# felixchenfy/Monocular-Visual-Odometry

Hardware: AMD Instinct MI355X
Metric: frames/sec (extract+match+5-kf BA), 640x480 / 2000 kp, 1->8 MI355X (higher is better)
Workload: dtype u8 (extract/match) + f64 (BA); 1 GPU

## Files before the change

monocular-visual-odometry_amd/csrc/ba_kernels.hip:

```cpp
#include "ba_types.h"
#include "mvo_internal.h"

typedef ba_u64 u64;
#ifndef MVO_KERNEL_SIM
typedef __attribute__((address_space(1))) double gdouble;
typedef __attribute__((address_space(1))) const u64 gcu64;
typedef __attribute__((address_space(1))) u64 gu64;
#define BA_AS_GLOBAL_D(p) ((gdouble*)(p))
#define BA_AS_GLOBAL_CU64(p) ((gcu64*)(p))
#define BA_AS_GLOBAL_U64(p) ((gu64*)(p))
#else
typedef double gdouble;
typedef const u64 gcu64;
typedef u64 gu64;
#define BA_AS_GLOBAL_D(p) (p)
#define BA_AS_GLOBAL_CU64(p) (p)
#define BA_AS_GLOBAL_U64(p) (p)
#endif

#define PH_BEGIN() long long ph_t = PROF ? (long long)__builtin_amdgcn_s_memtime() : 0
#define PH_END(id)                                                       \
    do {                                                                 \
        if (PROF) {                                                      \
            long long ph_n = (long long)__builtin_amdgcn_s_memtime();    \
// ... 344 lines not shown
    for (int o = 32; o > 0; o >>= 1) v = min(v, __shfl_xor(v, o));
    return v;
#endif
}

__device__ __forceinline__ int group_sum_i(int v, int width) {
#ifndef MVO_KERNEL_SIM
    v += __builtin_amdgcn_update_dpp(0, v, 0xb1, 0xf, 0xf, false);
    v += __builtin_amdgcn_update_dpp(0, v, 0x4e, 0xf, 0xf, false);
    if (width >= 8) v += __builtin_amdgcn_update_dpp(0, v, 0x141, 0xf, 0xf, false);
    if (width >= 16) v += __builtin_amdgcn_update_dpp(0, v, 0x140, 0xf, 0xf, false);
    return v;
#else
    for (int o = 1; o < width; o <<= 1) v += __shfl_xor(v, o);
    return v;
#endif
}

__device__ __attribute__((noinline)) void ba_pivot_replay(const short* rank, int n, short* perm, int lane) {
    const int done = 0x7fffffff;
    if (n <= 64) {
        int rk = lane < n ? (int)rank[lane] : -1, el = lane, out = 0, cur = 0;
        for (int k = 0; k < n; ++k) {
            const unsigned long long fresh = __ballot(rk == k), running = __ballot(rk == cur);
            const unsigned long long m = fresh ? fresh : running;
            cur = fresh ? k : cur;
            const int big = m ? (int)__builtin_ctzll(m) : k;
            const int kr = __builtin_amdgcn_readlane(rk, k), ke = __builtin_amdgcn_readlane(el, k), eb = __builtin_amdgcn_readlane(el, big);
            rk = lane == big ? kr : rk;
            el = lane == big ? ke : el;
            rk = lane == k ? -1 : rk;
            out = lane == k ? eb : out;
        }
        if (lane < n) perm[lane] = (short)out;
        return;
    }
    const int p0 = lane, p1 = lane + 64;
    int k0 = p0 < n ? ((int)rank[p0] << 7) | p0 : done, k1 = p1 < n ? ((int)rank[p1] << 7) | p1 : done;
    int e0 = p0, e1 = p1;
    for (int k = 0; k < n; ++k) {
        const int big = wave_min_i(min(k0, k1)) & 127;
        const int ek = k < 64 ? __builtin_amdgcn_readlane(e0, k) : __builtin_amdgcn_readlane(e1, k - 64);
        const int kk = k < 64 ? __builtin_amdgcn_readlane(k0, k) : __builtin_amdgcn_readlane(k1, k - 64);
        const int eb = big < 64 ? __builtin_amdgcn_readlane(e0, big) : __builtin_amdgcn_readlane(e1, big - 64);
        const int kmoved = (kk & ~127) | big;
        if (p0 == big) e0 = ek, k0 = kmoved;
        if (p1 == big) e1 = ek, k1 = kmoved;
        if (p0 == k) e0 = eb, k0 = done;
        if (p1 == k) e1 = eb, k1 = done;
    }
    if (p0 < n) perm[p0] = (short)e0;
    if (p1 < n) perm[p1] = (short)e1;
}

#include "ba_solve.h"

__device__ __attribute__((noinline)) double ba_stale_scale_landmarks(gcu64* dxl, int bl_off, int Lg, double lambda, int lane) {
    const double* bl = ba_dyn_lds + bl_off;
    double sp = 0;
    for (int l0 = lane; l0 < Lg; l0 += 4 * 64) {
        double xs[4][3];
#pragma unroll
        for (int u = 0; u < 4; ++u)
#pragma unroll
            for (int c = 0; c < 3; ++c) {
                const int l = l0 + 64 * u;
                xs[u][c] = l < Lg ? __longlong_as_double((long long)__hip_atomic_load(dxl + 3 * l + c, __ATOMIC_RELAXED, __HIP_MEMORY_SCOPE_AGENT)) : 0.0;
            }
#pragma unroll
        for (int u = 0; u < 4; ++u) {
            const int l = l0 + 64 * u;
            if (l < Lg) {
#pragma unroll
                for (int c = 0; c < 3; ++c) sp += xs[u][c] * (lambda * xs[u][c] + bl[3 * l + c]);
            }
        }
    }
    return wave_sum_d(sp);
}


__device__ __attribute__((noinline)) int solve_lds(int sl_off, int cb_off, int n, int lane) {
    double* S = ba_dyn_lds + sl_off;
    double* col = ba_dyn_lds + cb_off;
    const int ld = n + 2;
    int ok = 1;
    for (int j = 0; j < n; ++j) {
        const double d = S[j * ld + j];
        if (!(d >= BA_PIVOT_MIN && d <= BA_PIVOT_MAX)) {
            ok = 0;
            break;
        }
        const double r = ba_rcp_pivot(d);
        for (int i = j + 1 + lane; i <= n; i += 64) col[i] = S[i * ld + j];
        __builtin_amdgcn_wave_barrier();
        for (int i = j + 1 + lane; i <= n; i += 64) {
            const double l = col[i] * r;
            const int kend = i < n ? i : n - 1;
            for (int k = j + 1; k <= kend; ++k) S[i * ld + k] = __builtin_fma(-l, col[k], S[i * ld + k]);
            S[i * ld + j] = l;
        }
        __builtin_amdgcn_wave_barrier();
    }
    if (ok) {
        for (int j = lane; j < n; j += 64) col[j] = S[n * ld + j];
        __builtin_amdgcn_wave_barrier();
        for (int i = n - 1; i >= 1; --i) {
            const double xi = col[i];
            for (int j = lane; j < i; j += 64) col[j] = __builtin_fma(-S[i * ld + j], xi, col[j]);
            __builtin_amdgcn_wave_barrier();
        }
    }
    return ok;
}

__device__ __forceinline__ void packed_ij(int idx, int n, int& i, int& j) {
    const int ntri = n * (n + 1) / 2;
    if (idx < ntri) {
        i = (int)((sqrt(8.0 * idx + 1.0) - 1.0) * 0.5);
        while (i * (i + 1) / 2 > idx) --i;
        while ((i + 1) * (i + 2) / 2 <= idx) ++i;
        j = idx - i * (i + 1) / 2;
    } else {
        i = n;
        j = idx - ntri;
    }
}

struct WgLds {
    double* SL;
    double* colbuf;
    double* pan;
    double* Rl;
    double* hpl;
    double* uv;
    double* uvg;
    double* pts;
    double* bak;
    double* Hll;
    double* bl;
    double* Cc;
    double* cl;
    double* dxl;
    double* U;
    double* E2;
    short* epose;
    short* ept;
    short* dup;
    short* ptl;
    short* pti;
    short* pts0;
    short* eof;
};

__device__ __forceinline__ double edge_error(const BaDev& B, const WgLds& W, int el, const double* sR,
                                             const double* sT, double* Xc, double* ew) {
    const int p = W.epose[el], l = W.ept[el];
    const double* R = sR + 9 * p;
    const double* t = sT + 3 * p;
    const double X0 = W.pts[3 * l], X1 = W.pts[3 * l + 1], X2 = W.pts[3 * l + 2];
    Xc[0] = R[0] * X0 + R[1] * X1 + R[2] * X2 + t[0];
    Xc[1] = R[3] * X0 + R[4] * X1 + R[5] * X2 + t[1];
    Xc[2] = R[6] * X0 + R[7] * X1 + R[8] * X2 + t[2];
    const double mu = B.uv_global ? W.uvg[2 * el] : W.uv[el], mv = B.uv_global ? W.uvg[2 * el + 1] : W.uv[B.maxEg + el];
    const double e0 = mu - (Xc[0] / Xc[2] * B.f + B.cx);
    const double e1 = mv - (Xc[1] / Xc[2] * B.f + B.cy);
    ew[0] = B.lc00 * e0 + B.lc01 * e1;
    ew[1] = B.lc11 * e1;
    return ew[0] * ew[0] + ew[1] * ew[1];
}

__device__ double robust_chi2_local(const BaDev& B, const WgLds& W, int Eg, const double* sR, const double* sT,
                                    double* scratch) {
    double s = 0;
    for (int el = threadIdx.x; el < Eg; el += BA_THREADS) {
        double Xc[3], ew[2], r0, r1;
        huber(edge_error(B, W, el, sR, sT, Xc, ew), B.delta, r0, r1);
        s += r0;
    }
    return block_sum(s, scratch);
}

__device__ __forceinline__ int u_index(int col, int row, int ldu) {
    return col * ldu + row;
}

template <int LDU>
__device__ __forceinline__ v4d schur_chain_t(const double* U, int ti, int tj, int m0, int m1, int lane) {
    v4d acc = {0, 0, 0, 0};
    const int k = lane >> 4, i = lane & 15;
    constexpr int st = 4 * LDU;
    const double* pa = U + (size_t)(4 * m0 + k) * LDU + (16 * ti + i);
    const double* pb = U + (size_t)(4 * m0 + k) * LDU + (16 * tj + i);
    int m = m0;
#define BA_LOAD4(A, Bv) \
    A##0 = pa[0], Bv##0 = pb[0], A##1 = pa[st], Bv##1 = pb[st], A##2 = pa[2 * st], Bv##2 = pb[2 * st], A##3 = pa[3 * st], Bv##3 = pb[3 * st]; \
    pa += 4 * st;                                                                                                                           \
    pb += 4 * st
#define BA_MFMA4_LOADNEXT(A, Bv, C, D, more)                                     \
    acc = __builtin_amdgcn_mfma_f64_16x16x4f64(A##0, Bv##0, acc, 0, 0, 0);       \
    __builtin_amdgcn_sched_barrier(0);                                           \
    if (more) { BA_LOAD4(C, D); }                                                \
    __builtin_amdgcn_sched_barrier(0);                                           \
    acc = __builtin_amdgcn_mfma_f64_16x16x4f64(A##1, Bv##1, acc, 0, 0, 0);       \
    acc = __builtin_amdgcn_mfma_f64_16x16x4f64(A##2, Bv##2, acc, 0, 0, 0);       \
    acc = __builtin_amdgcn_mfma_f64_16x16x4f64(A##3, Bv##3, acc, 0, 0, 0)
    if (m + 4 <= m1) {
        double a0, a1, a2, a3, b0, b1, b2, b3, c0 = 0, c1 = 0, c2 = 0, c3 = 0, d0 = 0, d1 = 0, d2 = 0, d3 = 0;
        BA_LOAD4(a, b);
        m += 4;
        for (;;) {
            const bool more1 = m + 4 <= m1;
            BA_MFMA4_LOADNEXT(a, b, c, d, more1);
            if (!more1) break;
            m += 4;
            const bool more2 = m + 4 <= m1;
            BA_MFMA4_LOADNEXT(c, d, a, b, more2);
            if (!more2) break;
            m += 4;
        }
    }
#undef BA_LOAD4
#undef BA_MFMA4_LOADNEXT
    for (; m < m1; ++m) {
        acc = __builtin_amdgcn_mfma_f64_16x16x4f64(pa[0], pb[0], acc, 0, 0, 0);
        pa += st;
        pb += st;
    }
    return acc;
}
__device__ __forceinline__ v4d schur_chain(const double* U, int ldu, int ti, int tj, int m0, int m1, int lane) {
    switch (ldu) {
        case 17: return schur_chain_t<17>(U, ti, tj, m0, m1, lane);
        case 33: return schur_chain_t<33>(U, ti, tj, m0, m1, lane);
        case 49: return schur_chain_t<49>(U, ti, tj, m0, m1, lane);
        case 65: return schur_chain_t<65>(U, ti, tj, m0, m1, lane);
        default: break;
    }
    v4d acc = {0, 0, 0, 0};
    const int k = lane >> 4, i = lane & 15;
    const double* pa = U + (size_t)(4 * m0 + k) * ldu + (16 * ti + i);
    const double* pb = U + (size_t)(4 * m0 + k) * ldu + (16 * tj + i);
    for (int m = m0; m < m1; ++m) {
        acc = __builtin_amdgcn_mfma_f64_16x16x4f64(pa[0], pb[0], acc, 0, 0, 0);
        pa += 4 * ldu;
        pb += 4 * ldu;
    }
    return acc;
}

struct EdgeRegs {
    double a0[6], a1[6];
    double x[6];
};
__device__ __forceinline__ void edge_Y(const EdgeRegs& r, const double* cc, double* Y) {
    const double c0 = cc[0], c1 = cc[1], c2 = cc[2], c3 = cc[3], c4 = cc[4], c5 = cc[5];
    Y[0] = r.x[0] * c0 + r.x[1] * c1 + r.x[2] * c3;
    Y[1] = r.x[1] * c2 + r.x[2] * c4;
    Y[2] = r.x[2] * c5;
    Y[3] = r.x[3] * c0 + r.x[4] * c1 + r.x[5] * c3;
    Y[4] = r.x[4] * c2 + r.x[5] * c4;
    Y[5] = r.x[5] * c5;
}

struct BaRun {
    unsigned tag0;
    int use_mfma, same_l2_ok;
};
template <bool PROF, int NR, int SLOTS>
__device__ __forceinline__ void ba_window(const BaDev* desc, const BaRun batch, const int g) {
    __shared__ BaDev sB;
    {
        const unsigned* src = reinterpret_cast<const unsigned*>(desc);
        unsigned* dst = reinterpret_cast<unsigned*>(&sB);
        for (unsigned i = threadIdx.x; i < sizeof(BaDev) / 4; i += BA_THREADS) dst[i] = src[i];
    }
    __syncthreads();
    const BaDev& B = sB;
    if (g >= B.G) return;
    const unsigned long long t_begin = __builtin_amdgcn_s_memrealtime();
    double* dyn = ba_dyn_lds;
    __shared__ double sScr[BA_WAVES];
    double* const sP = dyn;
    double* const sPbak = sP + 8 * B.F;
    double* const sR = sPbak + 8 * B.F;
    double* const sT = sR + 9 * B.F;
    double* const sHpp = sT + 3 * B.F;
    double* const sBp = sHpp + 36 * B.F;
    double* const sDx = sBp + 6 * B.F;
    double* const sSol = sDx + 6 * B.F;
    double* const sX = dyn + ba_pose_doubles(B.F);
    __shared__ int sSlot[BA_MAX_POSES], sSlotPose[BA_MAX_POSES], sPoseStart[BA_MAX_POSES + 1];
    __shared__ short sSlc[3][BA_HP_PASSES][BA_MAX_POSES];
    __shared__ int sFlag[6];
    __shared__ double sStale[BA_WAVES + 2];
    __shared__ short sPermAll[2][6 * BA_MAX_POSES];
    short* const sPerm = sPermAll[0];
    __shared__ short sRank[6 * BA_MAX_POSES];
    short* const sPermTie = sPermAll[1];
    __shared__ long long sStamp[PROF ? 32 : 1];
    if (threadIdx.x == 0) sFlag[1] = sFlag[2] = sFlag[3] = sFlag[4] = 0;
    if (threadIdx.x < 6 * BA_MAX_POSES) sRank[threadIdx.x] = -1;
    int tid = threadIdx.x, lane = tid & 63;
#define BA_PHASE_HEAD()            \
    do {                           \
        tid = ba_fresh_i(tid);     \
        lane = tid & 63;           \
    } while (0)
    const int wave = __builtin_amdgcn_readfirstlane(tid >> 6);
    const int n = B.n, G = B.G, nfree = B.nfree, urows = B.ldu, ldu = B.ldu + 1, nlow = B.nlow, npk = B.npk;
    const int pt_lo = B.wg_pt_start[g], Lg = B.wg_pt_start[g + 1] - pt_lo;
    const int e_lo = B.wg_edge_start[g], Eg = B.wg_edge_start[g + 1] - e_lo;
    const unsigned tag0 = batch.tag0;
    unsigned tagA = 0, tagB = 0, tagH = 0;

    WgLds W;
    double* stage;
    {
        double* d = dyn + ba_pose_doubles(B.F) + 2 * (size_t)G + 8;
        W.SL = d;
        d += ba_solver_doubles(n, nlow + B.nhp, G, B.npair, B.npar, B.panel, B.alias_sl) - 3 * 64 - (B.panel ? BA_PANEL_DOUBLES : 0);
        W.colbuf = d;
        d += 3 * 64;
        W.pan = d;
        d += B.panel ? BA_PANEL_DOUBLES : 0;
        W.Rl = d;
        d += nlow + B.nhp + 16;
        W.hpl = d;
        d += B.nhp + 1;
        W.uv = d;
        d += B.uv_global ? 0 : (size_t)B.maxEg * 2;
        W.uvg = B.uv_dev + 2 * (size_t)e_lo;
        W.pts = d;
        d += (size_t)B.maxLg * 3;
        const size_t full = B.fix_points ? 0 : 1;
        W.bak = d;
        d += full * B.maxLg * 3;
        W.Hll = d;
        d += full * B.maxLg * BA_XS;
        W.bl = d;
        d += full * B.maxLg * 3;
        W.Cc = d;
        d += full * B.maxLg * BA_XS;
        W.cl = d;
        d += full * B.maxLg * 3;
        W.dxl = B.dxl_dev + 3 * (size_t)pt_lo;
        W.U = d;
        stage = d;
        if (B.alias_sl) W.SL = d;
        d += B.uarea;
        W.E2 = d;
        d += (size_t)B.e2_edges * BA_E2S;
        short* s = reinterpret_cast<short*>(d);
        W.epose = s;
        s += B.maxEg;
        W.ept = s;
        s += B.maxEg;
        W.dup = s;
        s += B.maxEg;
        W.ptl = s;
        s += B.maxEg;
        W.pti = s;
        s += B.maxEg;
        W.pts0 = s;
        s += B.maxLg + 1;
        W.eof = s;
    }
    for (int el = tid; el < Eg; el += BA_THREADS) {
        W.epose[el] = (short)B.e_pose[e_lo + el];
        W.ept[el] = (short)(B.e_point[e_lo + el] - pt_lo);
        W.dup[el] = B.dup_rank[e_lo + el];
        {
            const int pe = B.pt_edge_list[e_lo + el] - e_lo;
            W.ptl[el] = (short)pe;
            W.pti[pe] = (short)el;
        }
        if (B.uv_global) {
            W.uvg[2 * el] = B.e_uv[2 * (size_t)(e_lo + el)];
            W.uvg[2 * el + 1] = B.e_uv[2 * (size_t)(e_lo + el) + 1];
        } else {
            W.uv[el] = B.e_uv[2 * (size_t)(e_lo + el)];
            W.uv[B.maxEg + el] = B.e_uv[2 * (size_t)(e_lo + el) + 1];
        }
    }
    for (int i = tid; i < 3 * Lg; i += BA_THREADS) W.pts[i] = B.pts_in[3 * (size_t)pt_lo + i];
    if (!B.fix_points)
        for (int l = tid; l < Lg; l += BA_THREADS)
            BA_AS_GLOBAL_D(W.dxl)[3 * l] = BA_AS_GLOBAL_D(W.dxl)[3 * l + 1] = BA_AS_GLOBAL_D(W.dxl)[3 * l + 2] = 0.0;
    if (tid < 6 * B.F) sDx[tid] = 0.0;
    for (int i = tid; i <= Lg; i += BA_THREADS) W.pts0[i] = (short)(B.pt_edge_start[pt_lo + i] - e_lo);
    for (int i = tid; i < Lg * nfree; i += BA_THREADS) W.eof[i] = B.eof[(size_t)pt_lo * nfree + i];
    if (tid < B.F) {
        double Ri[9], ti[3], q[4];
        invert_Rt(B.poses_in + 16 * tid, Ri, ti);
        quat_from_R(Ri, q);
        quat_normalize(q);
        for (int i = 0; i < 4; ++i) sP[8 * tid + i] = q[i];
        for (int i = 0; i < 3; ++i) sP[8 * tid + 4 + i] = ti[i];
        quat_to_R(q, sR + 9 * tid);
        for (int i = 0; i < 3; ++i) sT[3 * tid + i] = ti[i];
        sSlot[tid] = B.pose_slot[tid];
    }
    if (tid < nfree) sSlotPose[tid] = B.slot_pose[tid];
    if (tid <= B.F) sPoseStart[tid] = B.wg_pose_start[g * (B.F + 1) + tid] - e_lo;
    __syncthreads();

    double lambda = 0, ni = 2;
    int it = 0, trials = 0, terminated = 0, error = 0, failed_solves = 0, stale_steps = 0;
    long long ph[PROF ? BA_NPHASE : 1] = {0};
    const long long ph_start = (long long)__builtin_amdgcn_s_memtime();
    double currentChi;
    bool same_l2 = false;
    bool grp_l2 = false;
    const int K = B.groups > 1 ? B.groups : 1;
    {
        double c = robust_chi2_local(B, W, Eg, sR, sT, sScr);
        if (G > 1) {
            ++tagB;
            u64* slot = B.xC + (size_t)(tagB & 1) * G * 4;
            const unsigned xcc = ba_xcc_id();
            if (tid == 0) {
                gstore_d(slot + 4 * g, tag0 + tagB, c, false);
                gstore_d(slot + 4 * g + 2, tag0 + tagB, (double)xcc, false);
            }
            if (!gather_tagged(slot, 2 * G, 2, 2, tag0 + tagB, sX)) sFlag[2] = 1;
            __syncthreads();
            if (sFlag[2]) error = 1;
            c = 0;
            bool one = true, grp = true;
            for (int w = 0; w < G; ++w) {
                c += sX[2 * w];
                one = one && sX[2 * w + 1] == sX[1];
                grp = grp && sX[2 * w + 1] == sX[2 * (w % K) + 1];
            }
            same_l2 = one && batch.same_l2_ok;
            grp_l2 = grp && batch.same_l2_ok;
            __syncthreads();
        }
        currentChi = c;
    }
    const double chi0 = currentChi;
    const bool any_free = nfree > 0 || !B.fix_points;
    const bool do_schur = !B.fix_points && n > 0;
    const int npar = B.npar, nseq = B.nseq;
    const int ncol = 3 * Lg;
    const int msteps = (ncol + 3) / 4;
    const int msplit = (msteps + B.nsplit - 1) / B.nsplit;
    const int chunk_cols = 4 * npar * msplit;
    const short* pkt_g = B.pk_of_tile;
    int pk4[4] = {-1, -1, -1, -1};
    if (do_schur && wave < B.npair * npar) {
#pragma unroll
        for (int j = 0; j < 4; ++j) pk4[j] = pkt_g[(wave % B.npair) * 256 + ((lane >> 4) + 4 * j) * 16 + (lane & 15)];
    }
    EdgeRegs er;
#pragma unroll
    for (int c = 0; c < 6; ++c) er.a0[c] = er.a1[c] = er.x[c] = 0;
    const bool have0 = SLOTS > 0 && tid < Eg, have1 = SLOTS > 1 && tid + BA_THREADS < Eg;
    const int e0_p = have0 ? W.epose[tid] : 0, e0_l = have0 ? W.ept[tid] : 0, e0_sl = have0 ? sSlot[e0_p] : -1;
    constexpr int nslot = SLOTS;
    constexpr int e2_first = SLOTS == 0 ? 0 : BA_THREADS;
#define BA_EDGE_FROM_LDS(BODY, el_)                                          \
    do {                                                                     \
        EdgeRegs r1_;                                                        \
        double ee_[2];                                                       \
        const double* q_ = W.E2 + BA_E2S * ((el_)-e2_first);                 \
        _Pragma("unroll") for (int c_ = 0; c_ < 6; ++c_) {                   \
            r1_.a0[c_] = q_[c_];                                             \
            r1_.a1[c_] = q_[6 + c_];                                         \
            r1_.x[c_] = q_[12 + c_];                                         \
        }                                                                    \
        ee_[0] = q_[18];                                                     \
        ee_[1] = q_[19];                                                     \
        const int p1_ = W.epose[el_];                                        \
        (void)p1_;                                                           \
        BODY(el_, r1_, W.ept[el_], sSlot[p1_], ee_)                          \
    } while (0);
#define BA_EDGES(BODY)                                                       \
    if (nslot > 0 && have0) do { BODY(tid, er, e0_l, e0_sl, ee0) } while (0); \
    if (nslot > 1 && have1) BA_EDGE_FROM_LDS(BODY, tid + BA_THREADS)         \
    if (nslot == 0)                                                          \
        for (int el0_ = tid; el0_ < Eg; el0_ += BA_THREADS) BA_EDGE_FROM_LDS(BODY, el0_)

    int hp_npass = 1;
    {
        const int mcap = (int)(B.uarea / BA_MSTRIDE);
        for (;; ++hp_npass) {
            int tot = 0;
            for (int p = 0; p < B.F; ++p) {
                const int n_p = sPoseStart[p + 1] - sPoseStart[p];
                tot += min(n_p, ((n_p + hp_npass - 1) / hp_npass + 1) & ~1);
            }
            if (tot <= mcap) break;
            if (hp_npass > Eg) {
                error = 1;
                break;
            }
        }
    }
    const bool hp_tables = hp_npass <= BA_HP_PASSES;
    auto hp_slice_row = [&](int q, int row) {
        if (tid < B.F) {
            int off = 0, lo = 0, hi = 0;
            for (int pp = 0; pp <= tid; ++pp) {
                const int s0 = sPoseStart[pp], n_p = sPoseStart[pp + 1] - s0;
                const int h = ((n_p + hp_npass - 1) / hp_npass + 1) & ~1;
                off += hi - lo;
                lo = min(s0 + q * h, s0 + n_p);
                hi = min(s0 + (q + 1) * h, s0 + n_p);
            }
            sSlc[0][row][tid] = (short)lo;
            sSlc[1][row][tid] = (short)hi;
            sSlc[2][row][tid] = (short)off;
        }
    };
    if (hp_tables && !error)
        for (int q = 0; q < hp_npass; ++q) hp_slice_row(q, q);
    int nfp = 0, hp_pa0 = -1, hp_pb0 = -1, hp_pa1 = -1, hp_pb1 = -1;
    for (int p = 0; p < B.F; ++p) {
        if (sSlot[p] < 0) continue;
        if (nfp == 2 * wave) hp_pa0 = p;
        if (nfp == 2 * wave + 1) hp_pb0 = p;
        if (nfp == 2 * (wave + BA_WAVES)) hp_pa1 = p;
        if (nfp == 2 * (wave + BA_WAVES) + 1) hp_pb1 = p;
        ++nfp;
    }
    __syncthreads();

    int piv_hoff = 0;
    if (NR == 32 && n > 0) {
        const int lsh = NR == 32 ? 4 : (n <= 32 ? 4 : (n <= 64 ? 3 : 2)), LPR = 1 << lsh, jj = tid & (LPR - 1);
        const int qi = min(tid >> lsh, n - 1), q0 = min(jj, n - 1), q1 = min(jj + LPR, n - 1);
        piv_hoff = (36 * sSlotPose[qi / 6] + 7 * (qi % 6)) | (36 * sSlotPose[q0 / 6] + 7 * (q0 % 6)) << 10 | (36 * sSlotPose[q1 / 6] + 7 * (q1 % 6)) << 20;
    }
    for (it = 0; any_free && !error && it < B.max_it; ++it) {
        PH_BEGIN();
        BA_PHASE_HEAD();
        double ee0[2] = {0, 0};
#define BA_LINEARIZE(el, r, p, sl, ee)                                                                              \
    {                                                                                                               \
        double Xc[3], ew[2], rho0_, rho1_;                                                                          \
        const double chi = edge_error(B, W, el, sR, sT, Xc, ew);                                                    \
        huber(chi, B.delta, rho0_, rho1_);                                                                          \
        const double sw = sqrt(rho1_);                                                                              \
        const double x = Xc[0], y = Xc[1], z = Xc[2], z2 = z * z, f = B.f;                                          \
        if (sl >= 0) {                                                                                              \
            const double J0[6] = {x * y / z2 * f, -(1 + (x * x / z2)) * f, y / z * f, -1. / z * f, 0, x / z2 * f};   \
            const double J1[6] = {(1 + y * y / z2) * f, -x * y / z2 * f, -x / z * f, 0, -1. / z * f, y / z2 * f};    \
            _Pragma("unroll") for (int c = 0; c < 6; ++c) {                                                         \
                r.a0[c] = sw * (B.lc00 * J0[c] + B.lc01 * J1[c]);                                                   \
                r.a1[c] = sw * (B.lc11 * J1[c]);                                                                    \
            }                                                                                                       \
        } else {                                                                                                    \
            _Pragma("unroll") for (int c = 0; c < 6; ++c) r.a0[c] = r.a1[c] = 0;                                    \
        }                                                                                                           \
        ee[0] = sw * ew[0];                                                                                         \
        ee[1] = sw * ew[1];                                                                                         \
        _Pragma("unroll") for (int c = 0; c < 6; ++c) r.x[c] = 0;                                                   \
        if (!B.fix_points) {                                                                                        \
            const double* R = sR + 9 * (p);                                                                         \
            const double t0[3] = {f, 0, -x / z * f}, t1[3] = {0, f, -y / z * f};                                    \
            _Pragma("unroll") for (int c = 0; c < 3; ++c) {                                                         \
                double j0 = -1. / z * (t0[0] * R[c] + t0[1] * R[3 + c] + t0[2] * R[6 + c]);                         \
                double j1 = -1. / z * (t1[0] * R[c] + t1[1] * R[3 + c] + t1[2] * R[6 + c]);                         \
                r.x[c] = sw * (B.lc00 * j0 + B.lc01 * j1);                                                          \
                r.x[3 + c] = sw * (B.lc11 * j1);                                                                    \
            }                                                                                                       \
        }                                                                                                           \
    }
        if (nslot > 0 && have0) BA_LINEARIZE(tid, er, e0_p, e0_sl, ee0)
        for (int el = nslot == 0 ? tid : tid + BA_THREADS; nslot != 1 && el < Eg; el += BA_THREADS) {
            EdgeRegs r1;
            double ee[2];
            const int p1 = W.epose[el], sl1 = sSlot[p1];
            BA_LINEARIZE(el, r1, p1, sl1, ee)
            double* q = W.E2 + BA_E2S * (el - e2_first);
#pragma unroll
            for (int c = 0; c < 6; ++c) {
                q[c] = r1.a0[c];
                q[6 + c] = r1.a1[c];
                q[12 + c] = r1.x[c];
            }
            q[18] = ee[0];
            q[19] = ee[1];
        }
        __syncthreads();
        PH_END(0);
        double maxdiag = 0;
        BA_PHASE_HEAD();
        if (!B.fix_points) {
            for (int h = 0; h < B.npt; ++h) {
                const int l_lo = (int)((long long)Lg * h / B.npt), l_hi = (int)((long long)Lg * (h + 1) / B.npt);
                const int k_lo = W.pts0[l_lo], k_hi = W.pts0[l_hi];
#define BA_BODY_STAGE_X(el, r, l_, sl_, ee)                                   \
    const int k_ = W.pti[el];                                                \
    if (k_ < k_lo || k_ >= k_hi) break;                                      \
    double* Xs = stage + BA_SXS * (k_ - k_lo);                               \
    _Pragma("unroll") for (int c = 0; c < 6; ++c) Xs[c] = r.x[c];            \
    Xs[6] = ee[0];                                                           \
    Xs[7] = ee[1];
                BA_EDGES(BA_BODY_STAGE_X)
                __syncthreads();
                for (int l = l_lo + tid; l < l_hi; l += BA_THREADS) {
                    double h6[6] = {0, 0, 0, 0, 0, 0}, b[3] = {0, 0, 0};
                    for (int k = W.pts0[l]; k < W.pts0[l + 1]; ++k) {
                        const double* X = stage + BA_SXS * (k - k_lo);
                        const double e0 = X[6], e1 = X[7];
                        h6[0] += X[0] * X[0] + X[3] * X[3];
                        h6[1] += X[0] * X[1] + X[3] * X[4];
                        h6[2] += X[0] * X[2] + X[3] * X[5];
                        h6[3] += X[1] * X[1] + X[4] * X[4];
                        h6[4] += X[1] * X[2] + X[4] * X[5];
                        h6[5] += X[2] * X[2] + X[5] * X[5];
                        b[0] -= X[0] * e0 + X[3] * e1;
                        b[1] -= X[1] * e0 + X[4] * e1;
                        b[2] -= X[2] * e0 + X[5] * e1;
                    }
#pragma unroll
                    for (int i = 0; i < 6; ++i) W.Hll[BA_XS * l + i] = h6[i];
#pragma unroll
                    for (int i = 0; i < 3; ++i) W.bl[3 * l + i] = b[i];
                    maxdiag = fmax(maxdiag, fmax(fabs(h6[0]), fmax(fabs(h6[3]), fabs(h6[5]))));
                }
                __syncthreads();
            }
        }
        PH_END(2);
        const bool hp_deferred = do_schur && G > 1 && it > 0;
        const bool hp_local = hp_deferred || G == 1;
        if (!hp_deferred) ++tagH;
        BA_PHASE_HEAD();
        {
            const int col = lane & 15;
            v4d accp0 = {0, 0, 0, 0}, accp1 = {0, 0, 0, 0};
            for (int q = 0; q < hp_npass && !error; ++q) {
                const int tq = hp_tables ? q : 0;
                if (!hp_tables) {
                    hp_slice_row(q, 0);
                    __syncthreads();
                }
#define BA_BODY_STAGE_M(el, r, l_, sl_, ee)                                   \
    const int p_ = W.epose[el];                                              \
    const int lo_ = sSlc[0][tq][p_], hi_ = sSlc[1][tq][p_];                  \
    if ((el) < lo_ || (el) >= hi_) break;                                    \
    double* Mr = stage + BA_MSTRIDE * (sSlc[2][tq][p_] + (el)-lo_);          \
    _Pragma("unroll") for (int c = 0; c < 6; ++c) {                          \
        Mr[c] = r.a0[c];                                                     \
        Mr[7 + c] = r.a1[c];                                                 \
    }                                                                        \
    Mr[6] = ee[0];                                                           \
    Mr[13] = ee[1];
                BA_EDGES(BA_BODY_STAGE_M)
                __syncthreads();
                const bool lastq = q == hp_npass - 1;
                if (batch.use_mfma) {
                    int ai = 0;
                    for (int pair = wave; 2 * pair < nfp; pair += BA_WAVES, ++ai) {
                        const int pa = ai == 0 ? hp_pa0 : hp_pa1, pb = ai == 0 ? hp_pb0 : hp_pb1;
                        const bool second = col >= 8;
                        const int pp = second ? pb : pa;
                        const int cc7 = col & 7;
                        const bool cv = cc7 < 7 && pp >= 0;
                        const int rowsA = 2 * (sSlc[1][tq][pa] - sSlc[0][tq][pa]);
                        const int rowsB = pb >= 0 ? 2 * (sSlc[1][tq][pb] - sSlc[0][tq][pb]) : 0;
                        const int s = pp >= 0 ? sSlc[2][tq][pp] : 0, rows = second ? rowsB : rowsA;
                        const int rmax = max(rowsA, rowsB);
                        const double* pm = stage + BA_MSTRIDE * (s + (lane >> 5)) + 7 * ((lane >> 4) & 1) + (cv ? cc7 : 0);
                        const int kq = lane >> 4;
                        const int myrows = cv ? rows - kq : 0;
                        v4d acc = ai == 0 ? accp0 : accp1;
                        int st = 0;
#define BA_HP_LOAD4(V)                                                                   \
    V##0 = 4 * st < myrows ? pm[0] : 0.0, V##1 = 4 * st + 4 < myrows ? pm[2 * BA_MSTRIDE] : 0.0, \
    V##2 = 4 * st + 8 < myrows ? pm[4 * BA_MSTRIDE] : 0.0, V##3 = 4 * st + 12 < myrows ? pm[6 * BA_MSTRIDE] : 0.0; \
    pm += 8 * BA_MSTRIDE;                                                                \
    st += 4
#define BA_HP_MFMA4_LOADNEXT(V, Wn, more)                                      \
    acc = __builtin_amdgcn_mfma_f64_16x16x4f64(V##0, V##0, acc, 0, 0, 0);       \
    __builtin_amdgcn_sched_barrier(0);                                          \
    if (more) { BA_HP_LOAD4(Wn); }                                              \
    __builtin_amdgcn_sched_barrier(0);                                          \
    acc = __builtin_amdgcn_mfma_f64_16x16x4f64(V##1, V##1, acc, 0, 0, 0);       \
    acc = __builtin_amdgcn_mfma_f64_16x16x4f64(V##2, V##2, acc, 0, 0, 0);       \
    acc = __builtin_amdgcn_mfma_f64_16x16x4f64(V##3, V##3, acc, 0, 0, 0)
                        if (4 * (st + 4) <= rmax) {
                            double a0, a1, a2, a3, c0 = 0, c1 = 0, c2 = 0, c3 = 0;
                            BA_HP_LOAD4(a);
                            for (;;) {
                                const bool more1 = 4 * (st + 4) <= rmax;
                                BA_HP_MFMA4_LOADNEXT(a, c, more1);
                                if (!more1) break;
                                const bool more2 = 4 * (st + 4) <= rmax;
                                BA_HP_MFMA4_LOADNEXT(c, a, more2);
                                if (!more2) break;
                            }
                        }
#undef BA_HP_LOAD4
#undef BA_HP_MFMA4_LOADNEXT
                        for (; 4 * st < rmax; ++st) {
                            const double v = 4 * st < myrows ? pm[0] : 0.0;
                            acc = __builtin_amdgcn_mfma_f64_16x16x4f64(v, v, acc, 0, 0, 0);
                            pm += 2 * BA_MSTRIDE;
                        }
                        if (ai == 0) accp0 = acc;
                        else accp1 = acc;
                        if (lastq) {
#pragma unroll
                            for (int j = 0; j < 4; ++j) {
                                const int rg = (lane >> 4) + 4 * j;
                                const bool mine = second ? (rg >= 8 && rg < 15 && pb >= 0) : rg < 7;
                                const int r7 = rg & 7;
                                if (mine && cc7 <= r7 && cc7 < 7) {
                                    const int sl = sSlot[pp], pk = r7 * (r7 + 1) / 2 + cc7;
                                    if (hp_local) W.hpl[BA_HP * sl + pk] = acc[j];
                                    else gstore_d(B.xH + 2 * ((size_t)g * B.nhp + BA_HP * sl + pk), tag0 + tagH, acc[j], same_l2);
                                }
                            }
                        }
                    }
                } else {
                    for (int p = wave; p < B.F; p += BA_WAVES) {
                        const int sl = sSlot[p];
                        if (sl < 0 || lane >= BA_HP) continue;
                        const int lo = sSlc[0][tq][p], hi = sSlc[1][tq][p];
                        const int s = sSlc[2][tq][p], e = s + hi - lo;
                        int i = 0;
                        while ((i + 1) * (i + 2) / 2 <= lane) ++i;
                        const int j = lane - i * (i + 1) / 2;
                        double acc = q == 0 ? 0.0 : W.hpl[BA_HP * sl + lane];
                        for (int r = 2 * s; r < 2 * e; ++r)
                            acc = __builtin_fma(stage[BA_MSTRIDE * (r >> 1) + 7 * (r & 1) + i], stage[BA_MSTRIDE * (r >> 1) + 7 * (r & 1) + j], acc);
                        if (hp_local || !lastq) W.hpl[BA_HP * sl + lane] = acc;
                        else gstore_d(B.xH + 2 * ((size_t)g * B.nhp + BA_HP * sl + lane), tag0 + tagH, acc, same_l2);
                    }
                }
                __syncthreads();
            }
        }
        PH_END(1);
        BA_PHASE_HEAD();
        if (!hp_deferred) {
            const double m = block_max(maxdiag, sScr);
            const int nhp = B.nhp, hrows = min(G, max(1, (int)(B.uarea / nhp)));
            double hsum = 0, mm = 0;
            if (G > 1) {
                if (tid == 0) gstore_d(B.xH + 2 * ((size_t)g * nhp + nhp - 1), tag0 + tagH, m, same_l2);
                for (int w0 = 0; w0 < G; w0 += hrows) {
                    const int nr = min(hrows, G - w0);
                    if (!gather_tagged(B.xH + 2 * (size_t)w0 * nhp, nr * nhp, nhp, nhp, tag0 + tagH, stage)) sFlag[2] = 1;
                    __syncthreads();
                    if (tid < nhp - 1) {
#pragma unroll 8
                        for (int w = 0; w < nr; ++w) hsum += stage[w * nhp + tid];
                    }
                    if (tid < nr) mm = fmax(mm, stage[tid * nhp + nhp - 1]);
                    __syncthreads();
                }
                if (sFlag[2]) error = 1;
            } else {
                if (tid < nhp - 1) hsum = W.hpl[tid];
                if (tid == 0) mm = m;
            }
            if (tid < BA_HP * nfree) {
                const int sl = tid / BA_HP, pk = tid - BA_HP * sl, p = sSlotPose[sl];
                int i = 0;
                while ((i + 1) * (i + 2) / 2 <= pk) ++i;
                const int j = pk - i * (i + 1) / 2;
                if (i < 6) {
                    sHpp[36 * p + 6 * i + j] = hsum;
                    sHpp[36 * p + 6 * j + i] = hsum;
                } else if (j < 6) {
                    sBp[6 * p + j] = -hsum;
                }
            }
            if (it == 0) {
                __syncthreads();
                if (tid < 6 * B.F && sSlot[tid / 6] >= 0) mm = fmax(mm, fabs(sHpp[36 * (tid / 6) + 7 * (tid % 6)]));
                lambda = 1e-5 * block_max(mm, sScr);
                ni = 2;
            }
            __syncthreads();
        }
        PH_END(2);

        double rho = 0;
        int qmax = 0;
        bool hp_pending = hp_deferred;
        do {
            STAMP(0);
            BA_PHASE_HEAD();
            int ist = nlow;
            if (!B.fix_points) {
                for (int l = tid; l < Lg; l += BA_THREADS) {
                    const double* h = W.Hll + BA_XS * l;
                    const double D[9] = {h[0] + lambda, h[1], h[2], h[1], h[3] + lambda, h[4], h[2], h[4], h[5] + lambda};
                    double Di[9];
                    inv3(D, Di);
                    const double c00 = sqrt(Di[0]), c10 = Di[3] / c00, c20 = Di[6] / c00;
                    const double c11 = sqrt(Di[4] - c10 * c10), c21 = (Di[7] - c20 * c10) / c11;
                    const double c22 = sqrt(Di[8] - c20 * c20 - c21 * c21);
                    double* cc = W.Cc + BA_XS * l;
                    cc[0] = c00;
                    cc[1] = c10;
                    cc[2] = c11;
                    cc[3] = c20;
                    cc[4] = c21;
                    cc[5] = c22;
                    const double* b = W.bl + 3 * l;
                    W.cl[3 * l] = c00 * b[0] + c10 * b[1] + c20 * b[2];
                    W.cl[3 * l + 1] = c11 * b[1] + c21 * b[2];
                    W.cl[3 * l + 2] = c22 * b[2];
                }
                __syncthreads();
            }
            STAMP(1);
            PH_END(3);
            BA_PHASE_HEAD();
            if (do_schur) {
                ++tagA;
                double* split_stage = W.SL;
                v4d run0 = {0, 0, 0, 0}, run1 = {0, 0, 0, 0};
                if (!batch.use_mfma)
                    for (int pk = tid; pk < nlow; pk += BA_THREADS) W.Rl[pk] = 0.0;
                const int nch = chunk_cols > 0 ? max(1, min(nseq, (4 * msteps + chunk_cols - 1) / chunk_cols)) : 1;
                for (int ch = 0; ch < nch; ++ch) {
                    const int c0 = ch * chunk_cols;
                    const int c1 = min(c0 + chunk_cols, 4 * msteps);
                    for (int q = tid; q < c1 - c0; q += BA_THREADS) {
                        const int colg = c0 + q;
                        double* uc = W.U + (size_t)q * ldu;
                        if (colg < ncol) {
                            uc[n] = W.cl[colg];
                        } else {
                            for (int row = 0; row <= n; ++row) uc[row] = 0.0;
                        }
                        for (int row = n + 1; row < urows; ++row) uc[row] = 0.0;
                    }
                    {
                        const int l0 = c0 / 3, l1 = min(Lg, (c1 + 2) / 3);
                        for (int q = l0 * nfree + tid; q < l1 * nfree; q += BA_THREADS) {
                            if (W.eof[q] >= 0) continue;
                            const int l = q / nfree, sl = q - l * nfree;
#pragma unroll
                            for (int k = 0; k < 3; ++k) {
                                const int colg = 3 * l + k;
                                if (colg < c0 || colg >= c1) continue;
#pragma unroll
                                for (int c = 0; c < 6; ++c) W.U[u_index(colg - c0, 6 * sl + c, ldu)] = 0.0;
                            }
                        }
                    }
                    if (PROF) {
                        __syncthreads();
                        STAMP(2);
                    }
#define BA_BODY_UFILL(el, r, l_, sl_, ee)                                                          \
    const int l = l_, sl = sl_;                                                                   \
    if (sl < 0 || 3 * l + 2 < c0 || 3 * l >= c1 || (has_dups && W.dup[el] != rank)) break;         \
    double Y[6];                                                                                  \
    edge_Y(r, W.Cc + BA_XS * l, Y);                                                               \
    _Pragma("unroll") for (int k = 0; k < 3; ++k) {                                               \
        const int colg = 3 * l + k;                                                               \
        if (!whole && (colg < c0 || colg >= c1)) continue;                                        \
        double* u = W.U + u_index(colg - c0, 6 * sl, ldu);                                        \
        _Pragma("unroll") for (int c = 0; c < 6; ++c) {                                           \
            const double v = r.a0[c] * Y[k] + r.a1[c] * Y[3 + k];                                 \
            if (has_dups && rank > 0) u[c] = u[c] + v;                                            \
            else u[c] = 0.0 + v;                                                                  \
        }                                                                                         \
    }
                    {
                        const bool has_dups = B.max_dup > 0;
                        const bool whole = c0 == 0 && c1 >= ncol;
                        for (int rank = 0; rank <= B.max_dup; ++rank) {
                            BA_EDGES(BA_BODY_UFILL)
                            __syncthreads();
                        }
                    }
                    STAMP(3);
// ... 619 lines not shown
```

Measured before the change: 5642 frames/s.

## Pack edge/landmark/slot indices and remap thread-to-edge assignment by point order

Packs each thread's edge index, landmark index and pose slot into one int kept in a register (slot 0) or in the E2 LDS record (slot 1). When the Schur chunked path is active, it assigns edges to threads through the point-ordered map ptl instead of the identity order. The goal is to cut repeated LDS index lookups and to make the threads handling a point's edges land together for the point-wise stages. It depends on a spare int slot at offset 20 in the E2 stride, bit-field limits (edge < 1024, landmark < 32768), and an extra indirection through W.epose during linearize.

```diff
diff --git a/monocular-visual-odometry_amd/csrc/ba_kernels.hip b/monocular-visual-odometry_amd/csrc/ba_kernels.hip
--- a/monocular-visual-odometry_amd/csrc/ba_kernels.hip
+++ b/monocular-visual-odometry_amd/csrc/ba_kernels.hip
@@ -670,10 +670,12 @@
     if (threadIdx.x == 0) sFlag[1] = sFlag[2] = sFlag[3] = sFlag[4] = 0;
     if (threadIdx.x < 6 * BA_MAX_POSES) sRank[threadIdx.x] = -1;
     int tid = threadIdx.x, lane = tid & 63;
+    int e0_pk = 0;
 #define BA_PHASE_HEAD()            \
     do {                           \
         tid = ba_fresh_i(tid);     \
         lane = tid & 63;           \
+        e0_pk = ba_fresh_i(e0_pk); \
     } while (0)
     const int wave = __builtin_amdgcn_readfirstlane(tid >> 6);
     const int n = B.n, G = B.G, nfree = B.nfree, urows = B.ldu, ldu = B.ldu + 1, nlow = B.nlow, npk = B.npk;
@@ -825,9 +827,37 @@
 #pragma unroll
     for (int c = 0; c < 6; ++c) er.a0[c] = er.a1[c] = er.x[c] = 0;
     const bool have0 = SLOTS > 0 && tid < Eg, have1 = SLOTS > 1 && tid + BA_THREADS < Eg;
-    const int e0_p = have0 ? W.epose[tid] : 0, e0_l = have0 ? W.ept[tid] : 0, e0_sl = have0 ? sSlot[e0_p] : -1;
+#define BA_EPK(el_) ((el_) | (int)W.ept[el_] << 10 | (sSlot[W.epose[el_]] + 1) << 25)
+#define BA_EPK_EDGE(pk_) ((pk_)&1023)
+#define BA_EPK_LANDMARK(pk_) (((pk_) >> 10) & 32767)
+#define BA_EPK_SLOT(pk_) (((pk_) >> 25) - 1)
+    const bool mapped = do_schur && chunk_cols > 0 && min(nseq, (4 * msteps + chunk_cols - 1) / chunk_cols) > 1;
+    if (have0) {
+        const int m0 = mapped ? W.ptl[tid] : tid;
+        e0_pk = BA_EPK(m0);
+    }
+    if (have1) {
+        const int m1 = mapped ? W.ptl[BA_THREADS + tid] : BA_THREADS + tid;
+        reinterpret_cast<int*>(W.E2 + BA_E2S * tid + 20)[0] = BA_EPK(m1);
+    }
     constexpr int nslot = SLOTS;
     constexpr int e2_first = SLOTS == 0 ? 0 : BA_THREADS;
+#define BA_EDGE_FROM_E2(BODY)                                                \
+    do {                                                                     \
+        EdgeRegs r1_;                                                        \
+        double ee_[2];                                                       \
+        const double* q_ = W.E2 + BA_E2S * tid;                              \
+        const int pk1_ = reinterpret_cast<const int*>(q_ + 20)[0];           \
+        _Pragma("unroll") for (int c_ = 0; c_ < 6; ++c_) {                   \
+            r1_.a0[c_] = q_[c_];                                             \
+            r1_.a1[c_] = q_[6 + c_];                                         \
+            r1_.x[c_] = q_[12 + c_];                                         \
+        }                                                                    \
+        ee_[0] = q_[18];                                                     \
+        ee_[1] = q_[19];                                                     \
+        const int me1_ = BA_EPK_EDGE(pk1_);                                  \
+        BODY(me1_, r1_, BA_EPK_LANDMARK(pk1_), BA_EPK_SLOT(pk1_), ee_)       \
+    } while (0);
 #define BA_EDGE_FROM_LDS(BODY, el_)                                          \
     do {                                                                     \
         EdgeRegs r1_;                                                        \
@@ -845,8 +875,11 @@
         BODY(el_, r1_, W.ept[el_], sSlot[p1_], ee_)                          \
     } while (0);
 #define BA_EDGES(BODY)                                                       \
-    if (nslot > 0 && have0) do { BODY(tid, er, e0_l, e0_sl, ee0) } while (0); \
-    if (nslot > 1 && have1) BA_EDGE_FROM_LDS(BODY, tid + BA_THREADS)         \
+    if (nslot > 0 && have0) do {                                             \
+        const int me0_ = BA_EPK_EDGE(e0_pk);                                 \
+        BODY(me0_, er, BA_EPK_LANDMARK(e0_pk), BA_EPK_SLOT(e0_pk), ee0)      \
+    } while (0);                                                             \
+    if (nslot > 1 && have1) BA_EDGE_FROM_E2(BODY)                            \
     if (nslot == 0)                                                          \
         for (int el0_ = tid; el0_ < Eg; el0_ += BA_THREADS) BA_EDGE_FROM_LDS(BODY, el0_)
 
@@ -936,13 +969,17 @@
             }                                                                                                       \
         }                                                                                                           \
     }
-        if (nslot > 0 && have0) BA_LINEARIZE(tid, er, e0_p, e0_sl, ee0)
-        for (int el = nslot == 0 ? tid : tid + BA_THREADS; nslot != 1 && el < Eg; el += BA_THREADS) {
+        if (nslot > 0 && have0) {
+            const int me0 = BA_EPK_EDGE(e0_pk), p0 = W.epose[me0], sl0 = BA_EPK_SLOT(e0_pk);
+            BA_LINEARIZE(me0, er, p0, sl0, ee0)
+        }
+        for (int s = nslot == 0 ? tid : tid + BA_THREADS; nslot != 1 && s < Eg; s += BA_THREADS) {
             EdgeRegs r1;
             double ee[2];
+            double* q = W.E2 + BA_E2S * (s - e2_first);
+            const int el = nslot == 0 ? s : BA_EPK_EDGE(reinterpret_cast<const int*>(q + 20)[0]);
             const int p1 = W.epose[el], sl1 = sSlot[p1];
             BA_LINEARIZE(el, r1, p1, sl1, ee)
-            double* q = W.E2 + BA_E2S * (el - e2_first);
 #pragma unroll
             for (int c = 0; c < 6; ++c) {
                 q[c] = r1.a0[c];
```

After: 5666 frames/s (median of 4 runs). About the same (+0.4%).
